# springmeyer/cov-tiles

Hardware: AMD Instinct MI355X
Metric: GB/s raw COVT bytes decoded + Mvertices/s, z2–z14 tile batch, 1/2/4/8 GPU (higher is better)
Workload: dtype int32

## Files before the change

### cov-tiles_amd/csrc/covt_decode.hip

```cpp
#include <hip/hip_runtime.h>
#include <stdint.h>

#include "covt.h"
#include "covt_internal.h"
#include "covt_wave.h"
#include "covt_walk.h"

namespace covt {

constexpr int kWin = 1024;

#ifndef COVT_LONG_STREAM
#define COVT_LONG_STREAM 16384
#endif
#ifndef COVT_LONG_PRIO
#define COVT_LONG_PRIO 2
#endif
#ifndef COVT_RLE_SHORT_SPAN
#define COVT_RLE_SHORT_SPAN 448
#endif
#ifndef COVT_CHUNK_PRIO
#define COVT_CHUNK_PRIO 2
#endif
constexpr int kLongStream = COVT_LONG_STREAM;
#ifdef COVT_TIMING
constexpr int kPhases = 8;
__device__ uint32_t* covt_phase_buf;
__device__ const covt_stream_desc* covt_phase_desc0;
#endif

typedef __attribute__((address_space(3))) const uint16_t lds_cu16;

struct __attribute__((aligned(16))) WaveSmem {
    int32_t misc[4];
    uint16_t cpre[64];
    uint16_t cmask[64];
    union alignas(16) {
        struct {
            uint32_t win[kWin / 4 + 4];
            uint16_t list[kWin];
            uint16_t next[kWin + 8];
            uint16_t grec[64];
        } v;
        struct {
            union {
                uint32_t stage[324];
                uint32_t ring[512];
            };
            uint32_t patch[256];
            uint32_t cbuf[260];
            union {
                uint8_t posx[2][192];
                uint32_t xw[224];
            };
        } f;
    } u;
};
constexpr int kSmemHdr = 272;
constexpr int kFamSmemRle = kSmemHdr + (kWin / 4 + 4) * 4 + kWin * 2 + (kWin + 8) * 2 + 64 * 2;
constexpr int kFamSmemVarint = kSmemHdr + (kWin / 4 + 4) * 4 + kWin * 2;
constexpr int kFamSmemFpf = kSmemHdr + (512 + 256 + 260 + 224) * 4 > kFamSmemVarint
                                ? kSmemHdr + (512 + 256 + 260 + 224) * 4
                                : kFamSmemVarint;
constexpr int kFpfXw = 224;
static_assert(kFamSmemFpf >= kSmemHdr + (int)sizeof(((WaveSmem*)nullptr)->u.f), "FastPFOR scratch stride");
static_assert(kFamSmemVarint >= kSmemHdr + (int)sizeof(((WaveSmem*)nullptr)->u.v.win) +
                                    (int)sizeof(((WaveSmem*)nullptr)->u.v.list), "varint scratch stride");
static_assert(__builtin_offsetof(WaveSmem, u) == kSmemHdr, "WaveSmem header size");
static_assert(kFamSmemRle == (int)sizeof(WaveSmem), "RLE uses the whole scratch");
static_assert(kFamSmemRle % 16 == 0 && kFamSmemVarint % 16 == 0 && kFamSmemFpf % 16 == 0, "16-B strides");

typedef uint32_t u32x4 __attribute__((ext_vector_type(4)));
typedef __attribute__((address_space(1))) const uint32_t g_u32;
typedef __attribute__((address_space(1))) const u32x4 g_v4;
__device__ __forceinline__ const g_u32* g32(uintptr_t a) { return (const g_u32*)a; }
__device__ __forceinline__ uint4 ld128(uintptr_t a16) {
    const u32x4 v = *(const g_v4*)a16;
    return make_uint4(v.x, v.y, v.z, v.w);
}
typedef __attribute__((address_space(1))) const uint8_t g_u8;
__device__ __forceinline__ uint4 ld128_off(const g_u8* base, uint32_t off) {
    const u32x4 v = *(const g_v4*)(base + off);
    return make_uint4(v.x, v.y, v.z, v.w);
}

__device__ __forceinline__ uint32_t ld_le32(const uint8_t* p) {
    const uintptr_t a = (uintptr_t)p;
    const g_u32* q = g32(a & ~(uintptr_t)3);
    return __builtin_amdgcn_alignbyte(q[1], q[0], (uint32_t)(a & 3));
}
__device__ __forceinline__ uint32_t ld_be32(const uint8_t* p) { return __builtin_bswap32(ld_le32(p)); }
__host__ __device__ constexpr uint32_t be_sel(uint32_t sh) {
    return (sh + 3u) | ((sh + 2u) << 8) | ((sh + 1u) << 16) | (sh << 24);
}
__device__ __forceinline__ uint32_t be_word(uint32_t hi, uint32_t lo, uint32_t sel) {
    return __builtin_amdgcn_perm(hi, lo, sel);
}
typedef __attribute__((address_space(4))) const uint32_t c_u32;
typedef __attribute__((address_space(4))) const u32x4 c_v4;
__device__ __forceinline__ uint32_t sld_le32(const uint8_t* p) {
    const uintptr_t a = (uintptr_t)p;
    const c_u32* q = (const c_u32*)(a & ~(uintptr_t)3);
    const uint64_t v = ((uint64_t)q[1] << 32) | q[0];
    return (uint32_t)(v >> (8u * (uint32_t)(a & 3u)));
}
__device__ __forceinline__ uint32_t sld_be32(const uint8_t* p) { return uniu(__builtin_bswap32(sld_le32(p))); }
__device__ __forceinline__ uint4 sld128(uintptr_t a16) {
    const u32x4 v = *(const c_v4*)a16;
    return make_uint4(v.x, v.y, v.z, v.w);
}

__device__ __forceinline__ uint32_t hibits4(uint32_t x) {
    x &= 0x80808080u;
    return ((x >> 7) & 1u) | ((x >> 14) & 2u) | ((x >> 21) & 4u) | ((x >> 28) & 8u);
}
__device__ __forceinline__ uint32_t hibits16(uint4 d) {
    return hibits4(d.x) | (hibits4(d.y) << 4) | (hibits4(d.z) << 8) | (hibits4(d.w) << 12);
}
__device__ __forceinline__ uint32_t range16(int32_t s, int32_t e) {
    s = s < 0 ? 0 : (s > 16 ? 16 : s);
    e = e < 0 ? 0 : (e > 16 ? 16 : e);
    if (e <= s) return 0u;
    return ((1u << e) - 1u) & ~((1u << s) - 1u);
}
typedef unsigned short u16x2 __attribute__((ext_vector_type(2)));
__device__ __forceinline__ uint32_t pext7(uint32_t x) {
    x &= 0x7f7f7f7fu;
    const uint32_t y = __builtin_bit_cast(uint32_t, __builtin_bit_cast(u16x2, x) >> (u16x2){1, 1});
    const uint32_t t = (x & 0x007f007fu) | (y & ~0x007f007fu);
    return (t & 0x3fffu) | ((t >> 2) & ~0x3fffu);
}
__device__ __forceinline__ uint32_t bytemask(int n) {
    return n >= 4 ? 0xffffffffu : (n <= 0 ? 0u : ((1u << (8 * n)) - 1u));
}
__device__ __forceinline__ int32_t zz32(uint32_t e) { return (int32_t)((e >> 1) ^ (0u - (e & 1u))); }
__device__ __forceinline__ int64_t zz64(uint64_t e) { return (int64_t)((e >> 1) ^ (0ull - (e & 1ull))); }

__host__ __device__ __forceinline__ void morton_xy(int32_t code, int nb, uint32_t& x, uint32_t& y) {
    uint32_t v = (uint32_t)code, t;
    t = (v ^ (v >> 1)) & 0x22222222u; v ^= t ^ (t << 1);
    t = (v ^ (v >> 2)) & 0x0c0c0c0cu; v ^= t ^ (t << 2);
    t = (v ^ (v >> 4)) & 0x00f000f0u; v ^= t ^ (t << 4);
    t = (v ^ (v >> 8)) & 0x0000ff00u; v ^= t ^ (t << 8);
    const uint32_t low = nb >= 16 ? 0xffffu : (nb <= 0 ? 0u : ((1u << nb) - 1u));
    const uint32_t top = nb <= 16 ? 0u : ((nb >= 32 ? 0xffffffffu : ((1u << nb) - 1u)) & ~0xffffu);
    const uint32_t hi = code < 0 ? top : 0u;
    x = (v & low) | hi;
// ... 19 lines not shown
#else
    __builtin_nontemporal_store(w, (i32x4*)p);
#endif
}
template <class T>
__device__ __forceinline__ void st_out(T* p, T v) {
#if defined(COVT_ABL_NOSTORE)
    *(T*)((uintptr_t)p & ~(uintptr_t)1023) = v;
#else
    *p = v;
#endif
}
__device__ __forceinline__ int64_t pack_xy(int32_t x, int32_t y) {
    return (int64_t)(((uint64_t)(uint32_t)y << 32) | (uint32_t)x);
}

template <int E>
__device__ __forceinline__ void store_run(uint8_t* arr, int32_t o, int32_t n, int64_t base, int32_t delta) {
    constexpr int K = 16 / E;
    const int l = lane_id();
    auto val = [&](int32_t i) -> int64_t { return (int64_t)((uint64_t)base + (uint64_t)(int64_t)(int32_t)(i * delta)); };
    const int32_t a0 = (o + K - 1) & ~(K - 1);
    const int32_t head = min(a0 - o, n);
    const int32_t nch = (n - head) / K;
    const int32_t body_end = head + nch * K;
    const int32_t ti = l < head ? l : body_end + (l - head);
    if (l < head || (l - head < n - body_end && l >= head)) {
        const int64_t v = val(ti);
        if (E == 8) st_out((int64_t*)arr + o + ti, v);
        else if (E == 4) st_out((int32_t*)arr + o + ti, (int32_t)v);
        else st_out(arr + o + ti, (uint8_t)v);
    }
    for (int32_t c0 = 0; c0 < nch; c0 += 64) {
        const int32_t ch = c0 + l < nch ? c0 + l : nch - 1;
        const int32_t i = head + K * ch;
        int4 w;
        if (E == 8) {
            const int64_t v0 = val(i), v1 = val(i + 1);
            w = make_int4((int)v0, (int)(v0 >> 32), (int)v1, (int)(v1 >> 32));
        } else if (E == 4) {
            w = make_int4((int)val(i), (int)val(i + 1), (int)val(i + 2), (int)val(i + 3));
        } else {
            const uint32_t b = (uint32_t)base & 0xffu, q = b * 0x01010101u;
            w = make_int4((int)q, (int)q, (int)q, (int)q);
        }
        st_out16((int32_t*)(arr + (int64_t)(o + i) * E), w);
    }
}

template <int E>
__device__ __forceinline__ void store_run_q(uint8_t* arr, int32_t o, int32_t n, int64_t base, int32_t delta) {
    constexpr int K = 16 / E;
    static_assert(2 * (K - 1) <= 16, "head and tail elements fit a quarter");
    const int q = lane_id() & 15;
    auto val = [&](int32_t i) -> int64_t { return (int64_t)((uint64_t)base + (uint64_t)(int64_t)(int32_t)(i * delta)); };
    const int32_t a0 = (o + K - 1) & ~(K - 1);
    const int32_t head = n > 0 ? min(a0 - o, n) : 0;
    const int32_t nch = n > 0 ? (n - head) / K : 0;
    const int32_t body_end = head + nch * K;
    const int32_t tailn = n > 0 ? n - body_end : 0;
    if (q < head + tailn) {
        const int32_t ti = q < head ? q : body_end + (q - head);
        const int64_t v = val(ti);
        if (E == 8) st_out((int64_t*)arr + o + ti, v);
        else st_out((int32_t*)arr + o + ti, (int32_t)v);
    }
    const int32_t steps = (int32_t)wave_max((uint32_t)((nch + 15) >> 4));
    for (int32_t c0 = 0; c0 < 16 * steps; c0 += 16) {
        const int32_t ch = c0 + q;
        if (ch < nch) {
            const int32_t i = head + K * ch;
            int4 w;
            if (E == 8) {
                const int64_t v0 = val(i), v1 = val(i + 1);
                w = make_int4((int)v0, (int)(v0 >> 32), (int)v1, (int)(v1 >> 32));
            } else {
                w = make_int4((int)val(i), (int)val(i + 1), (int)val(i + 2), (int)val(i + 3));
            }
            st_out16((int32_t*)(arr + (int64_t)(o + i) * E), w);
        }
    }
}

template <int OP, int K>
__device__ __forceinline__ void sink_values(const uint32_t (&vin)[K], int64_t base, int32_t first, int32_t count,
                                            int nb, uint8_t* __restrict__ out, Carry& c) {
    const int l = lane_id();
    const bool full = first == 0 && count >= 64 * K;
    const int32_t s0 = l * K - first;
    const bool lfull = full || (s0 >= 0 && s0 + K <= count);
    const int64_t i0 = base + (int64_t)l * K;
    bool ok[K];
    uint32_t v[K];
#pragma unroll
    for (int k = 0; k < K; ++k) {
        ok[k] = full || (s0 + k >= 0 && s0 + k < count);
        v[k] = ok[k] ? vin[k] : 0u;
    }
    auto st32 = [&](const int32_t (&r)[K]) {
        int32_t* o = (int32_t*)out + i0;
        if (K == 4 && lfull) {
            st_out16(o, make_int4(r[0], r[K > 1 ? 1 : 0], r[K > 2 ? 2 : 0], r[K > 3 ? 3 : 0]));
        } else {
#pragma unroll
            for (int k = 0; k < K; ++k)
                if (ok[k]) st_out(o + k, r[k]);
        }
    };
    auto st64 = [&](const int64_t (&r)[K]) {
        int64_t* o = (int64_t*)out + i0;
#pragma unroll
        for (int k = 0; k < K; ++k)
            if (ok[k]) st_out(o + k, r[k]);
    };
    if constexpr (OP == COVT_OP_VARINT_I32 || OP == COVT_OP_VARINT_ZZ_I32) {
        int32_t r[K];
#pragma unroll
        for (int k = 0; k < K; ++k) r[k] = OP == COVT_OP_VARINT_I32 ? (int32_t)v[k] : zz32(v[k]);
        st32(r);
    } else if constexpr (OP == COVT_OP_VARINT_I32_AS_I64 || OP == COVT_OP_VARINT_ZZ_I32_AS_I64) {
        int64_t r[K];
#pragma unroll
        for (int k = 0; k < K; ++k) r[k] = OP == COVT_OP_VARINT_I32_AS_I64 ? (int64_t)(int32_t)v[k] : (int64_t)zz32(v[k]);
        st64(r);
    } else if constexpr (OP == COVT_OP_VARINT_ZZ_DELTA_I32 || OP == COVT_OP_FPF_ZZ_DELTA_I32 ||
                         OP == COVT_OP_VARINT_ZZ_DELTA_I64) {
        uint32_t sacc[K];
        uint32_t acc = 0;
#pragma unroll
        for (int k = 0; k < K; ++k) {
            acc += (uint32_t)zz32(v[k]);
            sacc[k] = acc;
        }
        const uint32_t inc = incl_scan(acc);
        const uint32_t pre = c.x + inc - acc;
        if constexpr (OP == COVT_OP_VARINT_ZZ_DELTA_I64) {
            int64_t r[K];
#pragma unroll
            for (int k = 0; k < K; ++k) r[k] = (int64_t)(int32_t)(pre + sacc[k]);
            st64(r);
        } else {
            int32_t r[K];
#pragma unroll
            for (int k = 0; k < K; ++k) r[k] = (int32_t)(pre + sacc[k]);
            st32(r);
        }
        c.x += lane_bcast(inc, 63);
    } else if constexpr (OP == COVT_OP_VARINT_ZZ_DELTA_XY || OP == COVT_OP_FPF_ZZ_DELTA_XY) {
        uint32_t sx[K], sy[K];
        uint32_t ax = 0, ay = 0;
        const uint32_t par0 = (uint32_t)(i0 & 1);
#pragma unroll
        for (int k = 0; k < K; ++k) {
            const uint32_t z = (uint32_t)zz32(v[k]);
            const bool isx = ((par0 + k) & 1u) == 0;
            ax += isx ? z : 0u;
            ay += isx ? 0u : z;
            sx[k] = ax;
            sy[k] = ay;
        }
        const uint32_t incx = incl_scan(ax), incy = incl_scan(ay);
        const uint32_t prex = c.x + incx - ax, prey = c.y + incy - ay;
        int32_t r[K];
#pragma unroll
        for (int k = 0; k < K; ++k) r[k] = (int32_t)((((par0 + k) & 1u) == 0) ? (prex + sx[k]) : (prey + sy[k]));
        st32(r);
        c.x += lane_bcast(incx, 63);
        c.y += lane_bcast(incy, 63);
    } else if constexpr (OP == COVT_OP_VARINT_DELTA_MORTON || OP == COVT_OP_FPF_DELTA_MORTON) {
        uint32_t sacc[K];
        uint32_t acc = 0;
#pragma unroll
        for (int k = 0; k < K; ++k) {
            acc += v[k];
            sacc[k] = acc;
        }
        const uint32_t inc = incl_scan(acc);
        const uint32_t pre = c.x + inc - acc;
        const int32_t half = morton_half(nb);
        int32_t* o = (int32_t*)out + 2 * i0;
        int32_t xy[2 * K];
#pragma unroll
        for (int k = 0; k < K; ++k) {
            uint32_t mx, my;
            morton_xy((int32_t)(pre + sacc[k]), nb, mx, my);
            xy[2 * k] = (int32_t)(mx - (uint32_t)half);
            xy[2 * k + 1] = (int32_t)(my - (uint32_t)half);
        }
        if (K == 4 && lfull) {
            st_out16(o, make_int4(xy[0], xy[1], xy[K > 1 ? 2 : 0], xy[K > 1 ? 3 : 0]));
            st_out16(o + 4, make_int4(xy[K > 2 ? 4 : 0], xy[K > 2 ? 5 : 0], xy[K > 3 ? 6 : 0], xy[K > 3 ? 7 : 0]));
        } else {
#pragma unroll
            for (int k = 0; k < K; ++k)
                if (ok[k]) st_out((int64_t*)(o + 2 * k), pack_xy(xy[2 * k], xy[2 * k + 1]));
        }
        c.x += lane_bcast(inc, 63);
    }
}

enum { MODE_RAW = 0, MODE_WORDREV = 1 };
enum { VAL_J4 = 0, VAL_VB = 1, VAL_U64 = 2, VAL_U64_STRICT = 3, VAL_NONE = 4 };

__device__ __forceinline__ uint32_t win_byte(const WaveSmem& sm, int32_t j) {
    return ((const uint8_t*)sm.u.v.win)[j];
}
__device__ __forceinline__ void win_bytes12(const WaveSmem& sm, int32_t j, uint32_t& x0, uint32_t& x1,
                                            uint32_t& x2) {
    const int32_t d = j >> 2;
    const uint32_t sh = (uint32_t)(j & 3);
    const uint32_t w0 = sm.u.v.win[d], w1 = sm.u.v.win[d + 1], w2 = sm.u.v.win[d + 2], w3 = sm.u.v.win[d + 3];
    x0 = __builtin_amdgcn_alignbyte(w1, w0, sh);
    x1 = __builtin_amdgcn_alignbyte(w2, w1, sh);
    x2 = __builtin_amdgcn_alignbyte(w3, w2, sh);
}

struct Win {
    int32_t woff;
    int32_t K;
    int32_t p0;
    bool valid, serial;
    uint4 d;
    uint32_t cpre, cmsk;
};

template <int MODE, int VAL>
__device__ void win_load(WaveSmem& sm, const uint8_t* sb, Win& w, int32_t p, int32_t end, const uint32_t* lsrc = nullptr,
                         int32_t lw0 = 0) {
    const int l = lane_id();
    uint4 d;
    int32_t woff;
    if (MODE == MODE_RAW) {
        const uintptr_t a = ((uintptr_t)(sb + p)) & ~(uintptr_t)15;
        woff = uni((int32_t)((intptr_t)a - (intptr_t)sb));
// ... 888 lines not shown

struct FpfWords {
    const uint8_t* sb;
    int32_t nw;
    uintptr_t s_end;
    struct Raw {
        uint4 r;
        int32_t base;
        uint32_t sh;
    };
    __device__ __forceinline__ Raw issue(int32_t w) const {
        const uintptr_t addr = (uintptr_t)sb + 4u * (uint32_t)w;
        const uintptr_t a16 = addr & ~(uintptr_t)15;
        const uint32_t o = (uint32_t)(addr & 15u);
        const uint32_t lmax = s_end > a16 ? (uint32_t)((s_end - 1 - a16) >> 4) : 0u;
        Raw q;
        q.r = ld128_off((const g_u8*)a16, 16u * min((uint32_t)lane_id(), lmax));
        q.base = uni(w - (int32_t)(o >> 2));
        q.sh = o & 3u;
        return q;
    }
    __device__ __forceinline__ int32_t store(uint32_t* dst, const Raw& q) const {
        const int l = lane_id();
        const uint32_t nx = lane_next(q.r.x);
        const uint32_t sel = be_sel(q.sh);
        const int32_t wl = q.base + 4 * l;
        uint4 wv;
        wv.x = wl < nw ? be_word(q.r.y, q.r.x, sel) : 0u;
        wv.y = wl + 1 < nw ? be_word(q.r.z, q.r.y, sel) : 0u;
        wv.z = wl + 2 < nw ? be_word(q.r.w, q.r.z, sel) : 0u;
        wv.w = wl + 3 < nw ? be_word(nx, q.r.w, sel) : 0u;
        wave_sync();
        ((uint4*)dst)[l] = wv;
        wave_sync();
        return q.base;
    }
    __device__ __forceinline__ int32_t load(uint32_t* dst, int32_t w) const { return store(dst, issue(w)); }
};

__device__ __forceinline__ bool fpf_page_meta(Ctx& c, const FpfStream& s, int32_t p0, int32_t& ie) {
    if (p0 >= s.nw) { c.err = COVT_ERR_TRUNCATED; return false; }
    const int64_t ie0 = (int64_t)p0 + (int32_t)(p0 == 1 ? s.head1 : s.W.uniform(p0));
    if (ie0 < 0 || ie0 >= s.nw) { c.err = COVT_ERR_TRUNCATED; return false; }
    ie = (int32_t)ie0;
    return true;
}

struct FpfDirWords {
    const FpfWords& ld;
    const uint32_t* cbuf;
    int32_t mw0;
    uint32_t* spill;
    int32_t dbase = INT32_MIN / 2;
    __device__ __forceinline__ uint32_t operator()(int64_t w64) {
        const int32_t w = (int32_t)w64;
        if (w >= mw0 && w < mw0 + 255) return uniu(cbuf[w - mw0]);
        if (w < dbase || w >= dbase + 255) dbase = ld.load(spill, w);
        return uniu(spill[w - dbase]);
    }
};

struct FpfFields {
    int32_t b, ce, idx;
    int32_t bcoff;
    int32_t next;
};
__device__ __forceinline__ FpfFields fpf_fields(uint32_t hw, int32_t cur) {
    FpfFields f;
    f.b = (int32_t)(int8_t)(hw & 0xffu);
    f.ce = (int32_t)((hw >> 8) & 0xffu);
    const int32_t hasx = f.ce > 0 ? 1 : 0;
    f.idx = hasx ? (int32_t)(int8_t)((hw >> 16) & 0xffu) - f.b : 1;
    f.bcoff = cur + 2 + hasx;
    f.next = f.bcoff + f.ce;
    return f;
}
__device__ __forceinline__ uint32_t fpf_header_word(const uint32_t* cbuf, int32_t j) {
    return uniu(__builtin_amdgcn_alignbyte(cbuf[(j >> 2) + 1], cbuf[j >> 2], (uint32_t)j & 3u));
}

template <bool WRAP>
__device__ __forceinline__ void fpf_unpack(const uint32_t* words, int32_t w0, int32_t b, uint32_t (&v)[4]) {
    const int l = lane_id();
    const uint32_t mask = b == 32 ? 0xffffffffu : ((1u << b) - 1u);
    uint32_t bit = __umul24((uint32_t)(l & 7) * 4u, (uint32_t)b);
    const int32_t wb = (int32_t)__umul24((uint32_t)(l >> 3), (uint32_t)b) + w0;
#pragma unroll
    for (int k = 0; k < 4; ++k) {
        const int32_t wi = wb + (int32_t)(bit >> 5);
        const uint32_t lo = words[WRAP ? wi & 511 : wi], hi = words[WRAP ? (wi + 1) & 511 : wi + 1];
        v[k] = __builtin_amdgcn_alignbit(hi, lo, bit & 31u) & mask;
        bit += (uint32_t)b;
    }
}

__device__ __forceinline__ int32_t fpf_xword(int32_t k, uint32_t xs, uint32_t i, uint32_t& xbit) {
    const uint32_t bit = __umul24(i, (uint32_t)k);
    xbit = bit & 31u;
    return (int32_t)(xs + (bit >> 5));
}

template <class XPair, class Pos>
__device__ __forceinline__ void fpf_patch(WaveSmem& sm, const Words& W, int32_t b, int32_t ce, int32_t k, uint32_t xs,
                                          uint32_t xcur, XPair&& xpair, Pos&& pos, uint32_t (&v)[4]) {
    const int l = lane_id();
    const bool el = l < ce;
    const uint32_t pos0 = pos(0);
    uint32_t ex = 1u;
    if (k != 1) {
        uint32_t xbit, lo, hi;
        const int32_t wi = fpf_xword(k, xs, xcur + (uint32_t)l, xbit);
        xpair(wi, el, lo, hi);
        const uint32_t m = k == 32 ? 0xffffffffu : ((1u << k) - 1u);
        ex = __builtin_amdgcn_alignbit(hi, lo, xbit) & m;
    }
    atomicOr(&sm.u.f.patch[el ? pos0 : (uint32_t)(4 * l)], el ? ex << (b & 31) : 0u);
    if (ce > 64) {
        for (int q = 1; q < 4; ++q) {
            const int32_t e = l + 64 * q;
            if (e < ce) {
                const uint32_t ex2 = k == 1 ? 1u : xget(W, xs, k, xcur + (uint32_t)e);
                atomicOr(&sm.u.f.patch[pos(q)], ex2 << (b & 31));
            }
        }
    }
    wave_sync();
    const uint4 pt = ((const uint4*)sm.u.f.patch)[l];
    v[0] |= pt.x;
    v[1] |= pt.y;
    v[2] |= pt.z;
    v[3] |= pt.w;
}

template <int OP, class Sink>
__device__ __forceinline__ void fpf_tail_fill(Ctx& c, const FpfStream& s, int32_t p, int32_t mw0, bool fill, Sink&& sink) {
    int32_t decoded = s.L;
    if (!c.err && p < s.nw) {
        int32_t vpos = 4 * p;
        const int32_t base = s.L;
        Win w;
        w.valid = false;
        const bool tail_in = s.L > 0 && ((vpos & ~15) >> 2) >= mw0 && s.nw - mw0 <= 255;
        const int32_t got = varint_take<MODE_WORDREV, VAL_VB>(
            *c.sm, c.sb, w, vpos, 4 * s.nw, c.n - s.L, true, c.err,
            [&](const uint32_t (&lo)[1], const uint32_t (&hi)[1], int32_t vb, int32_t, int32_t count) {
                sink(lo, (int64_t)base + vb, count);
            },
            0, nullptr, 0, tail_in ? c.sm->u.f.cbuf : nullptr, mw0);
        decoded = s.L + got;
    }
    if (!c.err) {
        for (int32_t b = decoded; fill && b < c.n; b += 64) {
            const uint32_t vv[1] = {0};
            sink(vv, (int64_t)b, c.n - b < 64 ? c.n - b : 64);
        }
        if (OP == COVT_OP_FPF_ZZ_DELTA_XY && (c.n & 1)) c.err = COVT_ERR_COUNT_MISMATCH;
    }
}

struct FpfHdr {
    int32_t b, ce, idx;
    uint32_t xcur;
    int32_t bcoff;
    int32_t next;
};
struct FpfPre {
    uint4 raw;
    uint32_t pos;
    uint32_t x0, x1, x2;
};

typedef uint32_t u32x3 __attribute__((ext_vector_type(3)));
typedef __attribute__((address_space(1))) const u32x3 g_v3;
typedef uint32_t u32x2 __attribute__((ext_vector_type(2)));
typedef __attribute__((address_space(1))) const u32x2 g_v2;

template <int OP, int K>
__device__ __forceinline__ void sum_values(const uint32_t (&v)[K], int64_t base, int32_t count, uint32_t& ax,
                                           uint32_t& ay) {
    const int l = lane_id();
#pragma unroll
    for (int k = 0; k < K; ++k) {
        const bool ok = l * K + k < count;
        const uint32_t z = ok ? (OP == COVT_OP_FPF_DELTA_MORTON ? v[k] : (uint32_t)zz32(v[k])) : 0u;
        const bool odd = OP == COVT_OP_FPF_ZZ_DELTA_XY && ((base + l * K + k) & 1);
        ax += odd ? 0u : z;
        ay += odd ? z : 0u;
    }
}
template <int OP>
__device__ __forceinline__ void fpf_prime_stores(uint8_t* __restrict__ out, int64_t base) {
    const int64_t i0 = base + 4 * (int64_t)lane_id();
    const int4 z = make_int4(0, 0, 0, 0);
    if constexpr (OP == COVT_OP_FPF_DELTA_MORTON) {
        int4* o = (int4*)((int32_t*)out + 2 * i0);
        o[0] = z;
        o[1] = z;
    } else {
        *(int4*)((int32_t*)out + i0) = z;
    }
}
struct FpfSkip {
    int32_t done = -1;
    int32_t cur0, pk;
    int xc;
// ... 144 lines not shown
            int32_t cur0 = 0;
            if (jb0 > 0 && jb0 < nblocks && !c.err) {
                if (skip && skip->done == done) {
                    cur0 = skip->cur0;
                    pk = skip->pk;
                    xc_v = skip->xc;
                } else {
                    int32_t cur = 0, pkk = pk;
                    for (int32_t j = 0; j < jb0; ++j) {
                        if (!xin && (uint32_t)(cur - cbase) > (uint32_t)(1020 - 8)) chunk_load(cur);
                        const FpfFields f = fpf_fields(fpf_header_word(sm.u.f.cbuf, cur - cbase), cur);
                        pkk += 8 * f.b;
                        xc_v += (f.idx >= 2 && f.idx <= 32 && l == f.idx) ? f.ce : 0;
                        cur = f.next;
                        if (cur > bclen) { c.err = COVT_ERR_BAD_HEADER; break; }
                    }
                    cur0 = uni(cur);
                    pk = uni(pkk);
                    if (skip) {
                        skip->done = done;
                        skip->cur0 = cur0;
                        skip->pk = pk;
                        skip->xc = xc_v;
                    }
                }
                COVT_PHASE(c, 0);
            }
            auto block = [&](int32_t j, const FpfPre& pc, FpfPre& pn, int slot) {
                FpfHdr hc;
                hc.b = uni(h.b);
                hc.ce = uni(h.ce);
                hc.idx = uni(h.idx);
                hc.xcur = uniu(h.xcur);
                hc.bcoff = uni(h.bcoff);
                hc.next = uni(h.next);
                const int32_t pkc = uni(pk);
                const int32_t b = hc.b;
                const uint32_t o = (sbmis + 4u * (uint32_t)pkc) & 15u;
                const int32_t qoff = (int32_t)(o >> 2);
                {
                    uint4 raw2 = make_uint4(0, 0, 0, 0);
                    if (b == 32) {
                        const uintptr_t a16 = ((uintptr_t)c.sb + 4u * (uint32_t)pkc) & ~(uintptr_t)15;
                        raw2 = sld128(a16 + 1024);
                    }
                    const uint32_t nxt = lane_next(pc.raw.x, raw2.x);
                    uint4 wv;
                    wv.x = be_word(pc.raw.y, pc.raw.x, bsel);
                    wv.y = be_word(pc.raw.z, pc.raw.y, bsel);
                    wv.z = be_word(pc.raw.w, pc.raw.z, bsel);
                    wv.w = be_word(nxt, pc.raw.w, bsel);
                    ((uint4*)sm.u.f.stage)[l] = wv;
                    if (b == 32 && l == 0) {
                        uint4 w2;
                        w2.x = be_word(raw2.y, raw2.x, bsel);
                        w2.y = be_word(raw2.z, raw2.y, bsel);
                        w2.z = be_word(raw2.w, raw2.z, bsel);
                        w2.w = be_word(0u, raw2.w, bsel);
                        ((uint4*)sm.u.f.stage)[64] = w2;
                    }
                }
                if (hc.ce > 0) ((uint4*)sm.u.f.patch)[l] = make_uint4(0, 0, 0, 0);
                wave_sync();
                COVT_PHASE(c, 1);
                if (j + 1 < nblocks) {
                    c.err = walk(hc.next, h);
                    pk = pkc + 8 * b;
                    if (!c.err && pk + 8 * h.b > nw32) c.err = COVT_ERR_TRUNCATED;
                    if (c.err) return;
                }
                prefetch(h, pk, pn, slot ^ 1);
                COVT_PHASE(c, 2);
                uint32_t v[4];
                fpf_unpack<false>(sm.u.f.stage, qoff, b, v);
                COVT_PHASE(c, 3);
#if defined(COVT_ABL_NOEXC)
                if (false) {
#else
                if (hc.ce > 0) {
#endif
                    const int32_t k = hc.idx;
                    const uint32_t xs = k >= 2 ? (uint32_t)__builtin_amdgcn_readlane(xs_v, k) : 0u;
                    fpf_patch(
                        sm, W, b, hc.ce, k, xs, hc.xcur,
                        [&](int32_t wi, bool el, uint32_t& lo, uint32_t& hi) {
                            if (xin) {
                                const int32_t m = el ? wi - mw0 : 0;
                                lo = sm.u.f.cbuf[m];
                                hi = sm.u.f.cbuf[m + 1];
                            } else {
                                lo = wi < nw32 ? be_word(pc.x1, pc.x0, bsel) : 0u;
                                hi = wi + 1 < nw32 ? be_word(pc.x2, pc.x1, bsel) : 0u;
                            }
                        },
                        [&](int q) -> uint32_t { return q == 0 ? pc.pos : sm.u.f.posx[slot][64 * (q - 1) + l]; }, v);
                }
                COVT_PHASE(c, 4);
#if defined(COVT_ABL_NOSTORE)
                sink_values<OP, 4>(v, 0, 0, kFpfBlock, c.nb, c.out, cr);
#else
                if (sum_only)
                    sum_values<OP, 4>(v, (int64_t)done + (int64_t)j * kFpfBlock, kFpfBlock, ax, ay);
                else
                    sink_values<OP, 4>(v, (int64_t)done + (int64_t)j * kFpfBlock, 0, kFpfBlock, c.nb, c.out, cr);
#endif
                wave_sync();
                COVT_PHASE(c, 5);
            };
            FpfPre preB;
            if (jb0 < nblocks && !c.err) {
                c.err = walk(cur0, h);
                if (!c.err && pk + 8 * h.b > nw32) c.err = COVT_ERR_TRUNCATED;
                if (!c.err) {
                    prefetch(h, pk, pre, 0, !spec);
                    if (!sum_only) fpf_prime_stores<OP>(c.out, (int64_t)done + (int64_t)jb0 * kFpfBlock);
                    int32_t j = jb0;
                    do {
                        block(j, pre, preB, 0);
                        if (j + 1 < nblocks && !c.err) block(j + 1, preB, pre, 1);
                        j += 2;
                    } while (j < nblocks && !c.err);
                }
            }
            done += thissize;
            p = ie;
            if (done >= v1) break;
        }
    }
    if (has_end)
        fpf_tail_fill<OP>(c, S, p, mw0, !sum_only, [&](const uint32_t (&vals)[1], int64_t base, int32_t count) {
            if (sum_only) sum_values<OP, 1>(vals, base, count, ax, ay);
            else sink_values<OP, 1>(vals, base, 0, count, c.nb, c.out, cr);
        });
    COVT_PHASE(c, 7);
    c.consumed = c.byte_length;
    if (sum_only) {
        sums->x = lane_bcast(incl_scan(ax), 63);
        sums->y = lane_bcast(incl_scan(ay), 63);
    }
    if (fin) *fin = cr;
}

template <int OP>
__device__ __forceinline__ void run_fastpfor_stream(Ctx& c) {
    WaveSmem& sm = *c.sm;
    const int l = lane_id();
    const FpfStream S = fpf_stream_head(c);
    const Words& W = S.W;
    const int32_t nw32 = S.nw;
    const uint32_t bsel = S.bsel;
    const uintptr_t s_end = S.s_end;
    const int32_t L = S.L;
    const FpfWords ld{c.sb, nw32, s_end};
    Carry cr{0u, 0u};
    int32_t p = 1;
    int xs_v = 0, xz_v = -1, xc_v = 0;
    int32_t mw0 = 0;
    if (!c.err && nw32 > 0) {
        int32_t done = 0;
        while (!c.err && done < L) {
            done = uni(done);
            const int32_t thissize = uni((L - done) < kFpfPage ? (L - done) : kFpfPage);
            const int32_t p0 = uni(p);
            int32_t ie;
            if (!fpf_page_meta(c, S, p0, ie)) break;
            const FpfWords::Raw mq = ld.issue(ie);
            const uintptr_t pa = (uintptr_t)c.sb + 4u * (uint32_t)(p0 + 1);
            const uintptr_t A0 = pa & ~(uintptr_t)127;
            const uint32_t glast = s_end > A0 ? (uint32_t)((s_end - 1 - A0) & ~(uintptr_t)15) : 0u;
            const int32_t wbase = uni((int32_t)(p0 + 1) - (int32_t)((pa - A0) >> 2));
            uint4 R = ld128_off((const g_u8*)A0, min(16u * (uint32_t)l, glast));
            int32_t kst = 0;
            int32_t vend = wbase;
            uint32_t prev63 = 0u;
            mw0 = ld.store(sm.u.f.cbuf, mq);
            FpfContainer ct;
            c.err = fpf_page_container((int32_t)uniu(sm.u.f.cbuf[ie - mw0]), (int64_t)ie + 1, nw32, ct);
            if (c.err) break;
            xc_v = 0;
            const int32_t bc = (int32_t)ct.bc;
            int64_t ie64 = ct.bc + ct.bclen / 4;
            FpfDirWords dword{ld, sm.u.f.cbuf, mw0, sm.u.f.ring};
            xs_v = 0;
            xz_v = -1;
            c.err = fpf_directory(dword, nw32, ie64, [&](int32_t k, int64_t start, int32_t size) {
                xs_v = l == k ? (int)(uint32_t)start : xs_v;
                xz_v = l == k ? size : xz_v;
            });
            if (c.err) break;
            const bool xin = ie64 - mw0 <= 255;
            ie = (int32_t)(ie64 < nw32 ? ie64 : (int64_t)nw32);
            COVT_PHASE(c, 0);
            const int32_t nblocks = uni(thissize / kFpfBlock);
            const int32_t bclen = uni(ct.bclen);
            const uint8_t* cb8 = (const uint8_t*)sm.u.f.cbuf;
            const g_u8* cbyte = (const g_u8*)(c.sb + 4u * (uint32_t)bc);
            int32_t cbase = 4 * (mw0 - bc);
            auto chunk_load = [&](int32_t at) {
                cbase = 4 * (ld.load(sm.u.f.cbuf, bc + (at >> 2)) - bc);
            };
            bool fin = false;
            int32_t bneed = INT32_MAX;
            auto stage = [&]() {
                const int32_t k = uni(kst);
                const uint32_t nx = lane_next(R.x, 0u);
                const int32_t w0 = wbase + 256 * k + 4 * l;
                uint4 wv;
                wv.x = w0 < nw32 ? be_word(R.y, R.x, bsel) : 0u;
                wv.y = w0 + 1 < nw32 ? be_word(R.z, R.y, bsel) : 0u;
                wv.z = w0 + 2 < nw32 ? be_word(R.w, R.z, bsel) : 0u;
                wv.w = w0 + 3 < nw32 ? be_word(nx, R.w, bsel) : 0u;
                const int32_t fw = wbase + 256 * k - 1;
                const uint32_t fix = fw < nw32 ? be_word(lane_bcast(R.x, 0), prev63, bsel) : 0u;
                prev63 = lane_bcast(R.w, 63);
                const uint32_t ri = (uint32_t)(256 * k + 4 * l) & 511u;
                wave_sync();
                if (l < 63) {
                    *(uint4*)&sm.u.f.ring[ri] = wv;
                } else {
                    sm.u.f.ring[ri] = wv.x;
                    sm.u.f.ring[ri + 1] = wv.y;
                    sm.u.f.ring[ri + 2] = wv.z;
                }
                if (l == 0 && k > 0) sm.u.f.ring[(uint32_t)(256 * k - 1) & 511u] = fix;
                wave_sync();
                kst = k + 1;
                vend = wbase + 256 * (k + 1) - 1;
                if (!fin || vend < bneed)
                    R = ld128_off((const g_u8*)A0, min(1024u * (uint32_t)(k + 1) + 16u * (uint32_t)l, glast));
                wave_sync();
            };
            int32_t cur = 0, pk = (int32_t)p0 + 1;
            for (int32_t jbat = 0, nbat = 0; jbat < nblocks && !c.err; jbat += nbat) {
                jbat = uni(jbat);
                nbat = uni(min(64, nblocks - jbat));
                uint32_t hw_v = 0u;
                int32_t cur_v = bclen + 1;
                cur = uni(cur);
                cbase = uni(cbase);
                if (!xin && cur <= bclen && (uint32_t)(cur - cbase) > (uint32_t)(1020 - 258)) chunk_load(cur);
                for (int32_t g = 0; g < nbat; ++g) {
                    cur = uni(cur);
                    cbase = uni(cbase);
                    if (cur > bclen) break;
                    if (!xin && cur - cbase > 1020 - 8) {
                        nbat = g;
                        break;
                    }
                    const uint32_t hw = fpf_header_word(sm.u.f.cbuf, cur - cbase);
                    const int32_t nx = fpf_fields(hw, cur).next;
                    if (!xin && g > 0 && nx - cbase > 1020) {
                        nbat = g;
                        break;
                    }
                    hw_v = l == g ? hw : hw_v;
                    cur_v = l == g ? cur : cur_v;
                    cur = nx;
                }
                nbat = uni(nbat);
                if (nbat == 0) {
                    c.err = COVT_ERR_BAD_HEADER;
                    break;
                }
                COVT_PHASE(c, 1);
                const bool in = l < nbat;
                const FpfFields f_l = fpf_fields(hw_v, cur_v);
                const int32_t b_v = f_l.b, ce_v = f_l.ce, idx_v = f_l.idx;
                const bool hasx = ce_v > 0;
                const bool arr_k = hasx && idx_v >= 2 && idx_v <= 32;
                const bool arr = in && arr_k;
                int32_t xcur_v = 0;
                for (uint64_t todo = __ballot(arr); todo;) {
                    const int32_t kk = __builtin_amdgcn_readlane(idx_v, (int32_t)__builtin_ctzll(todo));
                    const bool mine = arr && idx_v == kk;
                    const uint32_t v = mine ? (uint32_t)ce_v : 0u;
                    const uint32_t s = incl_scan(v);
                    const int32_t base = __builtin_amdgcn_readlane(xc_v, kk);
                    xcur_v = mine ? base + (int32_t)(s - v) : xcur_v;
                    xc_v += l == kk ? (int32_t)lane_bcast(s, 63) : 0;
// ... 16 lines not shown
                        nok = (int32_t)__builtin_ctzll(fail);
                        ferr = __builtin_amdgcn_readlane(bad ? COVT_ERR_BAD_HEADER : COVT_ERR_TRUNCATED, nok);
                    }
                }
                COVT_PHASE(c, 2);
                fin = jbat + nbat >= nblocks || ferr != 0;
                bneed = nok > 0 ? uni(__builtin_amdgcn_readlane(pk_v + 8 * b_v, nok - 1)) : 0;
                if (jbat == 0) stage();
                struct Hdr {
                    int32_t b, ce, idx, pk, bcoff, xo;
                    uint32_t xcur;
                };
                int32_t xo_v = 255;
                if (!xin) {
                    const bool ab = arr && l < nok;
                    const int32_t k = ab ? idx_v : 2;
                    const uint32_t xs = (uint32_t)lane_get(xs_v, k);
                    const uint32_t b0 = __umul24((uint32_t)xcur_v, (uint32_t)k);
                    const uint32_t b1 = __umul24((uint32_t)(xcur_v + ce_v), (uint32_t)k);
                    const int32_t wlo = (int32_t)(xs + (b0 >> 5));
                    const int32_t wn = ab ? (int32_t)((b1 + 31u) >> 5) - (int32_t)(b0 >> 5) + 1 : 0;
                    const uint32_t winc = incl_scan((uint32_t)wn);
                    const int32_t wo = (int32_t)(winc - (uint32_t)wn);
                    const int32_t wend = (int32_t)winc;
                    xo_v = ab && wend <= kFpfXw ? wo : 255;
                    const int32_t tot = uni(min((int32_t)lane_bcast(winc, 63), kFpfXw));
                    const g_u8* sb4 = (const g_u8*)(((uintptr_t)c.sb) & ~(uintptr_t)3);
                    u32x2 d[4];
                    bool okw[4];
#pragma unroll
                    for (int r = 0; r < 4; ++r) {
                        const int32_t t = 64 * r + l;
                        int32_t lo = 0, hi = 64;
#pragma unroll
                        for (int s2 = 0; s2 < 7; ++s2) {
                            const int32_t mid = (lo + hi) >> 1;
                            const bool le = lane_get(wend, mid & 63) <= t;
                            const bool act = lo < hi;
                            lo = act && le ? mid + 1 : lo;
                            hi = act && !le ? mid : hi;
                        }
                        const int32_t g = min(lo, 63);
                        const int32_t w = lane_get(wlo, g) + (t - lane_get(wo, g));
                        okw[r] = t < tot && w < nw32;
                        d[r] = *(const g_v2*)(sb4 + 4u * (okw[r] ? (uint32_t)w : 0u));
                    }
#pragma unroll
                    for (int r = 0; r < 4; ++r)
                        if (64 * r + l < kFpfXw) sm.u.f.xw[64 * r + l] = okw[r] ? be_word(d[r].y, d[r].x, bsel) : 0u;
                    wave_sync();
                }
                const uint32_t f_v = (uint32_t)(b_v & 0xff) | ((uint32_t)ce_v << 8) | ((uint32_t)(idx_v & 0xff) << 16) |
                                     ((uint32_t)xo_v << 24);
                const int32_t bo_v = f_l.bcoff;
                auto rec = [&](int32_t g, Hdr& h) {
                    const uint32_t f = uniu((uint32_t)__builtin_amdgcn_readlane((int32_t)f_v, g));
                    h.b = (int32_t)(f & 0xffu);
                    h.ce = (int32_t)((f >> 8) & 0xffu);
                    h.idx = (int32_t)(int8_t)((f >> 16) & 0xffu);
                    h.xo = (int32_t)(f >> 24);
                    h.xcur = uniu((uint32_t)__builtin_amdgcn_readlane(xcur_v, g));
                    h.bcoff = uni(__builtin_amdgcn_readlane(bo_v, g));
                    h.pk = uni(__builtin_amdgcn_readlane(pk_v, g));
                };
                fpf_prime_stores<OP>(c.out, (int64_t)done + (int64_t)jbat * kFpfBlock);
                auto block = [&](int32_t g) {
                    Hdr hc;
                    rec(g, hc);
                    const int32_t b = hc.b;
                    if (uni(vend) < hc.pk + 8 * b) stage();
                    if (hc.ce > 0) ((uint4*)sm.u.f.patch)[l] = make_uint4(0, 0, 0, 0);
                    COVT_PHASE(c, 3);
                    uint32_t v[4];
                    {
                        const int32_t r0 = (hc.pk - wbase) & 511;
                        if (r0 + 8 * b <= 511) fpf_unpack<false>(sm.u.f.ring, r0, b, v);
                        else fpf_unpack<true>(sm.u.f.ring, r0, b, v);
                    }
                    COVT_PHASE(c, 4);
                    if (hc.ce > 0) {
                        const int32_t k = hc.idx;
                        const uint32_t xs = k >= 2 ? (uint32_t)__builtin_amdgcn_readlane(xs_v, k) : 0u;
                        fpf_patch(
                            sm, W, b, hc.ce, k, xs, hc.xcur,
                            [&](int32_t wi, bool el, uint32_t& lo, uint32_t& hi) {
                                if (xin) {
                                    const int32_t m = el ? wi - mw0 : 0;
                                    lo = sm.u.f.cbuf[m];
                                    hi = sm.u.f.cbuf[m + 1];
                                } else if (hc.xo != 255) {
                                    const int32_t w0 = (int32_t)(xs + (__umul24(hc.xcur, (uint32_t)k) >> 5));
                                    const int32_t m = el ? hc.xo + wi - w0 : 0;
                                    lo = sm.u.f.xw[m];
                                    hi = sm.u.f.xw[m + 1];
                                } else {
                                    lo = el && wi < nw32 ? W(wi) : 0u;
                                    hi = el && wi + 1 < nw32 ? W(wi + 1) : 0u;
                                }
                            },
                            [&](int q) -> uint32_t {
                                return q == 0 ? cb8[min(max(hc.bcoff - cbase + l, 0), 4 * 260 - 1)]
                                              : cbyte[(hc.bcoff + l + 64 * q) ^ 3];
                            },
                            v);
                    }
                    COVT_PHASE(c, 5);
                    sink_values<OP, 4>(v, (int64_t)done + (int64_t)(jbat + g) * kFpfBlock, 0, kFpfBlock, c.nb, c.out, cr);
                    wave_sync();
                    COVT_PHASE(c, 6);
                };
                for (int32_t g = 0; g < nok; ++g) {
                    g = uni(g);
                    block(g);
                }
                if (ferr) c.err = ferr;
            }
            done += thissize;
            p = ie;
        }
    }
    fpf_tail_fill<OP>(c, S, p, mw0, true, [&](const uint32_t (&vals)[1], int64_t base, int32_t count) {
        sink_values<OP, 1>(vals, base, 0, count, c.nb, c.out, cr);
    });
    COVT_PHASE(c, 7);
    c.consumed = c.byte_length;
}

template <int OP>
__device__ __forceinline__ void fpf_add_carry(uint8_t* out, int32_t v0, int32_t v1, Carry cr) {
    const uint32_t cx = cr.x, cy = OP == COVT_OP_FPF_ZZ_DELTA_XY ? cr.y : cr.x;
    if ((cx | cy) == 0u) return;
    __builtin_amdgcn_s_waitcnt(0x0f70);
    int32_t* o = (int32_t*)out;
    typedef __attribute__((address_space(1))) i32x4 g_i4;
    const int32_t nq = (v1 - v0) >> 2;
    const int32_t last = v0 + 4 * (nq > 0 ? nq - 1 : 0);
    constexpr int kDeep = 8;
    for (int32_t q0 = 0; q0 < nq; q0 += 64 * kDeep) {
        i32x4 v[kDeep];
#pragma unroll
        for (int k = 0; k < kDeep; ++k) v[k] = *(const g_i4*)(o + min(v0 + 4 * (q0 + 64 * k + lane_id()), last));
#pragma unroll
        for (int k = 0; k < kDeep; ++k) {
            const int32_t q = q0 + 64 * k + lane_id();
            if (q < nq)
                st_out16(o + v0 + 4 * q, make_int4((int32_t)((uint32_t)v[k].x + cx), (int32_t)((uint32_t)v[k].y + cy),
                                                   (int32_t)((uint32_t)v[k].z + cx), (int32_t)((uint32_t)v[k].w + cy)));
        }
    }
    const int32_t i = v0 + 4 * nq + lane_id();
    if (i < v1) o[i] = (int32_t)((uint32_t)o[i] + (((i - v0) & 1) ? cy : cx));
}

constexpr int kSplitSlots = COVT_SPLIT_SLOTS;
struct Agg {
    int32_t cnt;
    uint32_t sx, sy;
};
__device__ __forceinline__ Agg agg_cat(const Agg& a, const Agg& b, bool xy) {
    if (a.cnt < 0) return a;
    if (b.cnt < 0) return Agg{b.cnt, b.sx, (uint32_t)a.cnt + b.sy};
    const bool sw = xy && (a.cnt & 1);
    return Agg{a.cnt + b.cnt, a.sx + (sw ? b.sy : b.sx), a.sy + (sw ? b.sx : b.sy)};
}
typedef __attribute__((address_space(1))) uint64_t g_u64;
__device__ __forceinline__ void rec_publish(covt_stream_result* rec, const Agg& a, uint32_t tag) {
    if (lane_id() == 0) {
        g_u64* g = (g_u64*)rec;
        const uint64_t t = (uint64_t)tag << 32;
        __hip_atomic_store(g, t | (uint32_t)a.cnt, __ATOMIC_RELAXED, __HIP_MEMORY_SCOPE_AGENT);
        __hip_atomic_store(g + 1, t | a.sx, __ATOMIC_RELAXED, __HIP_MEMORY_SCOPE_AGENT);
        __hip_atomic_store(g + 2, t | a.sy, __ATOMIC_RELAXED, __HIP_MEMORY_SCOPE_AGENT);
    }
}
__device__ __forceinline__ bool rec_try(covt_stream_result* rec, uint32_t tag, Agg& a) {
    g_u64* g = (g_u64*)rec;
    const uint64_t x0 = __hip_atomic_load(g, __ATOMIC_RELAXED, __HIP_MEMORY_SCOPE_AGENT);
    const uint64_t x1 = __hip_atomic_load(g + 1, __ATOMIC_RELAXED, __HIP_MEMORY_SCOPE_AGENT);
    const uint64_t x2 = __hip_atomic_load(g + 2, __ATOMIC_RELAXED, __HIP_MEMORY_SCOPE_AGENT);
    const bool ok = (uint32_t)(x0 >> 32) == tag && (uint32_t)(x1 >> 32) == tag && (uint32_t)(x2 >> 32) == tag;
    a = Agg{(int32_t)(uint32_t)x0, (uint32_t)x1, (uint32_t)x2};
    return uniu(ok ? 1u : 0u) != 0u;
}
constexpr int kRecAgg = 1, kRecIncl = 4, kRecTicket = 7;
static_assert(kSplitSlots == 8, "split record layout");
constexpr uint32_t kSpinLimit = 1u << 22;
__device__ Agg lookback(covt_stream_result* res, int64_t t, int32_t chunk, bool xy, int32_t& err) {
    Agg acc{0, 0u, 0u};
    int64_t k = t - 1;
    uint32_t spins = 0;
// ... 868 lines not shown
```

Baseline: 662.3.

## Speed FastPFOR decode: narrow-width unpack, LDS exception rounds, constant XY parity

Adds a fast path in fpf_unpack for bit widths up to 8, where each lane does one aligned word read and four bitfield extracts, plus an early exit for width zero. Exception patching for blocks with more than 64 exceptions now reads exception words and positions from LDS-staged buffers through a shared round lambda, where it used to fetch per-element from global memory. The XY delta sink takes a compile-time even base parity for 4-value FPF blocks, which drops per-lane parity computation. The constant parity assumes block bases are always even, and the LDS position reads use clamped indices into the chunk buffer, which could misread data when exceptions go past the staged window.

```diff
diff --git a/cov-tiles_amd/csrc/covt_decode.hip b/cov-tiles_amd/csrc/covt_decode.hip
--- a/cov-tiles_amd/csrc/covt_decode.hip
+++ b/cov-tiles_amd/csrc/covt_decode.hip
@@ -63,6 +63,11 @@
                                 ? kSmemHdr + (512 + 256 + 260 + 224) * 4
                                 : kFamSmemVarint;
 constexpr int kFpfXw = 224;
+#if defined(COVT_FPF_RT_PARITY)
+constexpr bool kFpfEvenBase = false;
+#else
+constexpr bool kFpfEvenBase = true;
+#endif
 static_assert(kFamSmemFpf >= kSmemHdr + (int)sizeof(((WaveSmem*)nullptr)->u.f), "FastPFOR scratch stride");
 static_assert(kFamSmemVarint >= kSmemHdr + (int)sizeof(((WaveSmem*)nullptr)->u.v.win) +
                                     (int)sizeof(((WaveSmem*)nullptr)->u.v.list), "varint scratch stride");
@@ -248,7 +253,7 @@
     }
 }
 
-template <int OP, int K>
+template <int OP, int K, bool EVEN = false>
 __device__ __forceinline__ void sink_values(const uint32_t (&vin)[K], int64_t base, int32_t first, int32_t count,
                                             int nb, uint8_t* __restrict__ out, Carry& c) {
     const int l = lane_id();
@@ -315,7 +320,7 @@
     } else if constexpr (OP == COVT_OP_VARINT_ZZ_DELTA_XY || OP == COVT_OP_FPF_ZZ_DELTA_XY) {
         uint32_t sx[K], sy[K];
         uint32_t ax = 0, ay = 0;
-        const uint32_t par0 = (uint32_t)(i0 & 1);
+        const uint32_t par0 = EVEN && K % 2 == 0 ? 0u : (uint32_t)(i0 & 1);
 #pragma unroll
         for (int k = 0; k < K; ++k) {
             const uint32_t z = (uint32_t)zz32(v[k]);
@@ -1370,6 +1375,22 @@
 template <bool WRAP>
 __device__ __forceinline__ void fpf_unpack(const uint32_t* words, int32_t w0, int32_t b, uint32_t (&v)[4]) {
     const int l = lane_id();
+#if !defined(COVT_FPF_WIDE_UNPACK)
+    if (b == 0) {
+#pragma unroll
+        for (int k = 0; k < 4; ++k) v[k] = 0u;
+        return;
+    }
+    if (b <= 8) {
+        const uint32_t o = __umul24((uint32_t)(l & 7) * 4u, (uint32_t)b);
+        const int32_t wi = (int32_t)__umul24((uint32_t)(l >> 3), (uint32_t)b) + w0 + (int32_t)(o >> 5);
+        const uint32_t lo = words[WRAP ? wi & 511 : wi], hi = words[WRAP ? (wi + 1) & 511 : wi + 1];
+        const uint32_t f = __builtin_amdgcn_alignbit(hi, lo, o & 31u);
+#pragma unroll
+        for (int k = 0; k < 4; ++k) v[k] = __builtin_amdgcn_ubfe(f, (uint32_t)(k * b), (uint32_t)b);
+        return;
+    }
+#endif
     const uint32_t mask = b == 32 ? 0xffffffffu : ((1u << b) - 1u);
     uint32_t bit = __umul24((uint32_t)(l & 7) * 4u, (uint32_t)b);
     const int32_t wb = (int32_t)__umul24((uint32_t)(l >> 3), (uint32_t)b) + w0;
@@ -1390,25 +1411,39 @@
 
 template <class XPair, class Pos>
 __device__ __forceinline__ void fpf_patch(WaveSmem& sm, const Words& W, int32_t b, int32_t ce, int32_t k, uint32_t xs,
-                                          uint32_t xcur, XPair&& xpair, Pos&& pos, uint32_t (&v)[4]) {
+                                          uint32_t xcur, bool xlds, XPair&& xpair, Pos&& pos, uint32_t (&v)[4]) {
     const int l = lane_id();
-    const bool el = l < ce;
-    const uint32_t pos0 = pos(0);
-    uint32_t ex = 1u;
-    if (k != 1) {
-        uint32_t xbit, lo, hi;
-        const int32_t wi = fpf_xword(k, xs, xcur + (uint32_t)l, xbit);
-        xpair(wi, el, lo, hi);
-        const uint32_t m = k == 32 ? 0xffffffffu : ((1u << k) - 1u);
-        ex = __builtin_amdgcn_alignbit(hi, lo, xbit) & m;
-    }
-    atomicOr(&sm.u.f.patch[el ? pos0 : (uint32_t)(4 * l)], el ? ex << (b & 31) : 0u);
+    const uint32_t m = k == 32 ? 0xffffffffu : ((1u << (k & 31)) - 1u);
+    auto round = [&](int q) {
+        const int32_t e = l + 64 * q;
+        const bool el = e < ce;
+        const uint32_t p = pos(q);
+        uint32_t ex = 1u;
+        if (k != 1) {
+            uint32_t xbit, lo, hi;
+            const int32_t wi = fpf_xword(k, xs, xcur + (uint32_t)e, xbit);
+            xpair(wi, el, lo, hi);
+            ex = __builtin_amdgcn_alignbit(hi, lo, xbit) & m;
+        }
+        atomicOr(&sm.u.f.patch[el ? p : (uint32_t)(4 * l)], el ? ex << (b & 31) : 0u);
+    };
+    round(0);
+#if defined(COVT_FPF_XROUNDS_MEM)
+    xlds = false;
+#endif
     if (ce > 64) {
-        for (int q = 1; q < 4; ++q) {
-            const int32_t e = l + 64 * q;
-            if (e < ce) {
-                const uint32_t ex2 = k == 1 ? 1u : xget(W, xs, k, xcur + (uint32_t)e);
-                atomicOr(&sm.u.f.patch[pos(q)], ex2 << (b & 31));
+        if (xlds) {
+            const int32_t nr = (ce + 63) >> 6;
+#pragma unroll
+            for (int q = 1; q < 4; ++q)
+                if (q < nr) round(q);
+        } else {
+            for (int q = 1; q < 4; ++q) {
+                const int32_t e = l + 64 * q;
+                if (e < ce) {
+                    const uint32_t ex2 = k == 1 ? 1u : xget(W, xs, k, xcur + (uint32_t)e);
+                    atomicOr(&sm.u.f.patch[pos(q)], ex2 << (b & 31));
+                }
             }
         }
     }
@@ -1719,7 +1754,7 @@
                     const int32_t k = hc.idx;
                     const uint32_t xs = k >= 2 ? (uint32_t)__builtin_amdgcn_readlane(xs_v, k) : 0u;
                     fpf_patch(
-                        sm, W, b, hc.ce, k, xs, hc.xcur,
+                        sm, W, b, hc.ce, k, xs, hc.xcur,  xin,
                         [&](int32_t wi, bool el, uint32_t& lo, uint32_t& hi) {
                             if (xin) {
                                 const int32_t m = el ? wi - mw0 : 0;
@@ -1739,7 +1774,7 @@
                 if (sum_only)
                     sum_values<OP, 4>(v, (int64_t)done + (int64_t)j * kFpfBlock, kFpfBlock, ax, ay);
                 else
-                    sink_values<OP, 4>(v, (int64_t)done + (int64_t)j * kFpfBlock, 0, kFpfBlock, c.nb, c.out, cr);
+                    sink_values<OP, 4, kFpfEvenBase>(v, (int64_t)done + (int64_t)j * kFpfBlock, 0, kFpfBlock, c.nb, c.out, cr);
 #endif
                 wave_sync();
                 COVT_PHASE(c, 5);
@@ -1831,7 +1866,9 @@
             const int32_t nblocks = uni(thissize / kFpfBlock);
             const int32_t bclen = uni(ct.bclen);
             const uint8_t* cb8 = (const uint8_t*)sm.u.f.cbuf;
+#if defined(COVT_FPF_XROUNDS_MEM)
             const g_u8* cbyte = (const g_u8*)(c.sb + 4u * (uint32_t)bc);
+#endif
             int32_t cbase = 4 * (mw0 - bc);
             auto chunk_load = [&](int32_t at) {
                 cbase = 4 * (ld.load(sm.u.f.cbuf, bc + (at >> 2)) - bc);
@@ -2014,7 +2051,7 @@
                         const int32_t k = hc.idx;
                         const uint32_t xs = k >= 2 ? (uint32_t)__builtin_amdgcn_readlane(xs_v, k) : 0u;
                         fpf_patch(
-                            sm, W, b, hc.ce, k, xs, hc.xcur,
+                            sm, W, b, hc.ce, k, xs, hc.xcur,  true,
                             [&](int32_t wi, bool el, uint32_t& lo, uint32_t& hi) {
                                 if (xin) {
                                     const int32_t m = el ? wi - mw0 : 0;
@@ -2031,13 +2068,16 @@
                                 }
                             },
                             [&](int q) -> uint32_t {
-                                return q == 0 ? cb8[min(max(hc.bcoff - cbase + l, 0), 4 * 260 - 1)]
-                                              : cbyte[(hc.bcoff + l + 64 * q) ^ 3];
+#if defined(COVT_FPF_XROUNDS_MEM)
+                                if (q) return cbyte[(hc.bcoff + l + 64 * q) ^ 3];
+#endif
+                                return cb8[min(max(hc.bcoff - cbase + l + 64 * q, 0), 4 * 260 - 1)];
                             },
                             v);
                     }
                     COVT_PHASE(c, 5);
-                    sink_values<OP, 4>(v, (int64_t)done + (int64_t)(jbat + g) * kFpfBlock, 0, kFpfBlock, c.nb, c.out, cr);
+                    sink_values<OP, 4, kFpfEvenBase>(v, (int64_t)done + (int64_t)(jbat + g) * kFpfBlock, 0, kFpfBlock, c.nb, c.out,
+                                                     cr);
                     wave_sync();
                     COVT_PHASE(c, 6);
                 };
```

Result: no change. 666.8, median of 2 (+0.7%).
